# yxlllc/DDSP-SVC

Hardware: AMD Instinct MI355X
Metric: audio samples/sec, CombSub 44.1kHz 256-harm hop512 (higher is better)
Workload: dtype f32; 1 GPU; combsub B=32/GPU x 10 s utterances (F=862, T=441344), n_mag 256/256/256, sr 44100, hop 512, DSP path (HOT-1 + HOT-2) from resident f0 / raw controls ~N(0,1) / uniform noise, signal only; batch_per_gpu=32, frames=862, samples_per_utterance=441344, parallelism=utterance-shard x1

## Files before the change

ddsp_svc_amd/csrc/frame_phase.h:

```cpp
#pragma once
#include "ddsp_common.h"

namespace ddsp {

template <int SPL>
struct FramePhase {
  float x[SPL];
  float f0u[SPL];
};

template <int SPL, bool POW2 = false>
__device__ __forceinline__ void frame_phase(const float* __restrict__ f0_row, int f, int hop, const Upsampler& up,
                                            const PhaseCfg& cfg, double phase0, float ip, int lane,
                                            FramePhase<SPL>& o) {
  double pre[SPL];
  double acc = 0.0;
  const Upsampler::Row3 rows = up.load3(f0_row, f);
#pragma unroll
  for (int r = 0; r < SPL; ++r) {
    int j = lane * SPL + r;
    float v = 0.f;
    if (j < hop) {
      v = POW2 ? up.at3_pow2(rows, j) : up.at3_in_frame(rows, j, hop);
      acc += cfg.term(v);
    }
    o.f0u[r] = v;
    pre[r] = acc;
  }
  double base = phase0 + wave_excl_scan(acc, lane);
#pragma unroll
  for (int r = 0; r < SPL; ++r) o.x[r] = cfg.wrap(base + pre[r], ip);
}

template <int SPL>
__device__ __forceinline__ void store_frame(float* __restrict__ dst, int hop, int lane, const float (&v)[SPL]) {
  if ((hop & 3) == 0 && ((reinterpret_cast<uintptr_t>(dst) & 15) == 0)) {
#pragma unroll
    for (int r = 0; r < SPL; r += 4) {
      int j = lane * SPL + r;
      if (j < hop) *reinterpret_cast<float4*>(dst + j) = make_float4(v[r], v[r + 1], v[r + 2], v[r + 3]);
    }
  } else {
#pragma unroll
    for (int r = 0; r < SPL; ++r) {
      int j = lane * SPL + r;
      if (j < hop) dst[j] = v[r];
    }
  }
}

template <int SPL, bool POW2>
__device__ __forceinline__ void combtooth_frame(const float* __restrict__ f0_frames, const float* __restrict__ initial_phase,
                                                long fr, int F, int hop, const Upsampler& up, const PhaseCfg& cfg,
                                                const double* __restrict__ phase0, float* __restrict__ out, int lane) {
  const unsigned bu = (unsigned)fr / (unsigned)F;
  const long b = bu;
  const int f = (int)((unsigned)fr - bu * (unsigned)F);
  const float ip = cfg.has_ip ? initial_phase[b] : 0.0f;
  FramePhase<SPL> ph;
  frame_phase<SPL, POW2>(f0_frames + b * F, f, hop, up, cfg, phase0[fr], ip, lane, ph);
  float v[SPL];
#pragma unroll
  for (int r = 0; r < SPL; ++r) {
    float num = cfg.sr_f * ph.x[r];
    float den = ph.f0u[r] + 1e-3f;
    v[r] = sinc_f32(div_pos(num, den));
  }
  store_frame<SPL>(out + fr * (long)hop, hop, lane, v);
}

}
```

Baseline: 50.02 billion samples/s.

## Use fixed-point 64-bit integer phase accumulation with DPP wave scan

Adds a fast path for inference mode that replaces the per-frame double-precision phase cumulative sum and wrap with a 48-bit fixed-point integer accumulation. Each f0 sample is converted via a magic-number FMA, and the prefix is computed with a DPP-based 64-bit inclusive wave scan. The scan no longer needs the double-precision wave_excl_scan, and the wrap becomes a bit shift instead of floor and subtraction. If any lane sees out-of-range f0 or phase, the whole wave falls back to the old double path. This adds a ballot, and it assumes that wrap semantics and the j<hop guard (now removed from the fast loop) match when the upsampler returns zero-safe values past hop.

```diff
diff --git a/ddsp_svc_amd/csrc/frame_phase.h b/ddsp_svc_amd/csrc/frame_phase.h
--- a/ddsp_svc_amd/csrc/frame_phase.h
+++ b/ddsp_svc_amd/csrc/frame_phase.h
@@ -32,6 +32,55 @@
   for (int r = 0; r < SPL; ++r) o.x[r] = cfg.wrap(base + pre[r], ip);
 }
 
+template <int CTRL, int ROW_MASK, bool BOUND>
+__device__ __forceinline__ unsigned long long dpp_u64(unsigned long long v) {
+  const unsigned lo = (unsigned)__builtin_amdgcn_update_dpp(0, (int)(unsigned)v, CTRL, ROW_MASK, 0xF, BOUND);
+  const unsigned hi = (unsigned)__builtin_amdgcn_update_dpp(0, (int)(unsigned)(v >> 32), CTRL, ROW_MASK, 0xF, BOUND);
+  return ((unsigned long long)hi << 32) | lo;
+}
+__device__ __forceinline__ unsigned long long wave_incl_scan_u64(unsigned long long v) {
+  v += dpp_u64<0x111, 0xF, true>(v);
+  v += dpp_u64<0x112, 0xF, true>(v);
+  v += dpp_u64<0x114, 0xF, true>(v);
+  v += dpp_u64<0x118, 0xF, true>(v);
+  v += dpp_u64<0x142, 0xA, false>(v);
+  v += dpp_u64<0x143, 0xC, false>(v);
+  return v;
+}
+
+template <int SPL, bool POW2 = false>
+__device__ __forceinline__ bool frame_phase_fx(const float* __restrict__ f0_row, int f, int hop, const Upsampler& up,
+                                               const PhaseCfg& cfg, double phase0, float ip, int lane, FramePhase<SPL>& o) {
+  const Upsampler::Row3 rows = up.load3(f0_row, f);
+  double b = phase0;
+  if (cfg.has_ip) b = b + ((double)ip / 2.0) / kPiD;
+  const double fb = b - rint(b);
+  const float lim = 4.0f * cfg.sr_f;
+  const bool ok = fabsf(rows.a) < lim && fabsf(rows.b) < lim && fabsf(rows.c) < lim && fabs(fb) <= 0.5;
+  if (__ballot(!ok)) return false;
+  const double magic = 6755399441055744.0;
+  const double k48 = cfg.rsr_d * 281474976710656.0;
+  unsigned long long pre[SPL];
+  unsigned long long acc = 0;
+#pragma unroll
+  for (int r = 0; r < SPL; ++r) {
+    const int j = lane * SPL + r;
+    const float v = POW2 ? up.at3_pow2(rows, j) : up.at3_in_frame(rows, j, hop);
+    acc += __builtin_bit_cast(unsigned long long, fma((double)v, k48, magic));
+    o.f0u[r] = v;
+    pre[r] = acc;
+  }
+  const unsigned long long base = __builtin_bit_cast(unsigned long long, fma(fb, 281474976710656.0, magic)) + (1ull << 15) +
+                                  (wave_incl_scan_u64(acc) - acc);
+#pragma unroll
+  for (int r = 0; r < SPL; ++r) {
+    const unsigned long long s = base + pre[r];
+    const int w = (int)(unsigned)(s >> 16);
+    o.x[r] = (float)w * 2.3283064365386963e-10f;
+  }
+  return true;
+}
+
 template <int SPL>
 __device__ __forceinline__ void store_frame(float* __restrict__ dst, int hop, int lane, const float (&v)[SPL]) {
   if ((hop & 3) == 0 && ((reinterpret_cast<uintptr_t>(dst) & 15) == 0)) {
@@ -58,7 +107,9 @@
   const int f = (int)((unsigned)fr - bu * (unsigned)F);
   const float ip = cfg.has_ip ? initial_phase[b] : 0.0f;
   FramePhase<SPL> ph;
-  frame_phase<SPL, POW2>(f0_frames + b * F, f, hop, up, cfg, phase0[fr], ip, lane, ph);
+  const double p0 = phase0[fr];
+  if (!cfg.infer || !frame_phase_fx<SPL, POW2>(f0_frames + b * F, f, hop, up, cfg, p0, ip, lane, ph))
+    frame_phase<SPL, POW2>(f0_frames + b * F, f, hop, up, cfg, p0, ip, lane, ph);
   float v[SPL];
 #pragma unroll
   for (int r = 0; r < SPL; ++r) {
```

Measured after the change: 50.71 billion samples/s (median of 6 runs). 1.4% higher.
